# LPengYang/MotionClone

Hardware: NVIDIA H100
Metric: frames/sec at 16x512x512 T2V, 50-step DDIM (higher is better)
Workload: dtype f16

## Files before the change

### motionclone_b200/csrc/spatial_attn_bwd_tc.cu

```cuda
#include <math.h>

#include "tma_common.cuh"

namespace mc {

constexpr int kBM = 128;
constexpr int kBT = 64;

struct FABwdParams {
  const float* lse2;
  const float* dsc;
  __half *dq, *dk, *dv;
  int64_t g_sb, g_sr;
  int B, Nq, Nk, H, Npad;
  float scale, scale_log2e;
};


template <int DH>
__global__ void __launch_bounds__(256) attn_bwd_prep_kernel(const __half* __restrict__ o, const __half* __restrict__ d_o,
                                                            const float* __restrict__ lse, float* __restrict__ lse2,
                                                            float* __restrict__ dsc, int64_t o_sb, int64_t o_sr,
                                                            int64_t do_sb, int64_t do_sr, int B, int N, int Npad, int H,
                                                            float scale) {
  const int64_t i = (int64_t)blockIdx.x * blockDim.x + threadIdx.x;
  if (i >= (int64_t)B * Npad * H) return;
  const int h = (int)(i % H);
  const int64_t br = i / H;
  const int r = (int)(br % Npad), b = (int)(br / Npad);
  const int64_t dst = ((int64_t)b * H + h) * Npad + r;
  if (r >= N) {
    lse2[dst] = 0.f, dsc[dst] = 0.f;
    return;
  }
  const uint4* po = reinterpret_cast<const uint4*>(o + b * o_sb + (int64_t)r * o_sr + h * DH);
  const uint4* pd = reinterpret_cast<const uint4*>(d_o + b * do_sb + (int64_t)r * do_sr + h * DH);
  float acc = 0.f;
#pragma unroll
  for (int c = 0; c < DH / 8; ++c) {
    const uint4 a = po[c], g = pd[c];
    const __half2* ah = reinterpret_cast<const __half2*>(&a);
    const __half2* gh = reinterpret_cast<const __half2*>(&g);
#pragma unroll
    for (int j = 0; j < 4; ++j) {
      const float2 x = __half22float2(ah[j]), y = __half22float2(gh[j]);
      acc = fmaf(x.x, y.x, acc);
      acc = fmaf(x.y, y.y, acc);
    }
  }
  lse2[dst] = lse[((int64_t)b * H + h) * N + r] * 1.44269504088896340736f;
  dsc[dst] = acc * scale;
}


template <int DH>
__device__ __forceinline__ void store_acc_rows(const float* acc, __half* base, int64_t sr, int row0, int nrows, int t) {
#pragma unroll
  for (int r = 0; r < 2; ++r) {
    const int row = row0 + 8 * r;
    if (row >= nrows) continue;
    __half* p = base + (int64_t)row * sr;
#pragma unroll
    for (int i = 0; i < AccW<DH>::REGS / 4; ++i) {
      const int col = 8 * i + 2 * t;
      if (col < DH) *reinterpret_cast<uint32_t*>(p + col) = pack_half2(acc[4 * i + 2 * r], acc[4 * i + 2 * r + 1]);
    }
  }
}

template <int DH, bool SINGLE>
struct DQCfg {
  static constexpr int BN = SINGLE ? kMaxTextKeys : kBT;
  using TQ = TileParts<DH, kBM>;
  using TK = TileParts<DH, BN>;
  static constexpr int ACC = AccW<DH>::REGS;
  static constexpr int NS = SINGLE ? 1 : 2;
  static constexpr int THREADS = 2 * 128 + 32;
  static constexpr int QB = align1k(TQ::BYTES), KB = align1k(TK::BYTES);
  static constexpr int OFF_Q = 0, OFF_DO = QB, OFF_K = 2 * QB, OFF_V = OFF_K + NS * KB, OFF_BAR = OFF_V + NS * KB;
  static constexpr int SMEM = OFF_BAR + 256 + 1024;
};

template <int DH, bool SINGLE, bool RAGGED>
__global__ void __launch_bounds__(DQCfg<DH, SINGLE>::THREADS, 1)
attn_bwd_dq_kernel(const __grid_constant__ CUtensorMap mq128, const __grid_constant__ CUtensorMap mq32,
                   const __grid_constant__ CUtensorMap mdo128, const __grid_constant__ CUtensorMap mdo32,
                   const __grid_constant__ CUtensorMap mk128, const __grid_constant__ CUtensorMap mk32,
                   const __grid_constant__ CUtensorMap mv128, const __grid_constant__ CUtensorMap mv32,
                   const FABwdParams prm) {
  using X = DQCfg<DH, SINGLE>;
  using TQ = typename X::TQ;
  using TK = typename X::TK;
  constexpr int BN = X::BN, NS = X::NS;

  extern __shared__ uint8_t smem_raw[];
  uint8_t* smem = reinterpret_cast<uint8_t*>((reinterpret_cast<uintptr_t>(smem_raw) + 1023) & ~(uintptr_t)1023);
  uint8_t* sQ = smem + X::OFF_Q;
  uint8_t* sDO = smem + X::OFF_DO;
  uint8_t* sK = smem + X::OFF_K;
  uint8_t* sV = smem + X::OFF_V;
  uint64_t* bars = reinterpret_cast<uint64_t*>(smem + X::OFF_BAR);
  uint64_t* bar_q = bars;
  uint64_t* full = bars + 1;
  uint64_t* empty = bars + 1 + NS;

  const int tid = threadIdx.x, warp = tid >> 5, lane = tid & 31;
  const int h = blockIdx.y, b = blockIdx.z;
  const int q0 = blockIdx.x * kBM;
  const int T_tiles = (prm.Nk + BN - 1) / BN;

  if (tid == 0) {
    mbar_init(bar_q, 1);
    for (int i = 0; i < NS; ++i) mbar_init(full + i, 1), mbar_init(empty + i, 8);
    fence_mbar_init();
  }
  __syncthreads();

  if (warp == 8) {
    if (lane == 0) {
      mbar_arrive_expect_tx(bar_q, 2 * TQ::BYTES);
      tma_load_tile<DH, kBM>(sQ, &mq128, &mq32, bar_q, q0, h, b);
      tma_load_tile<DH, kBM>(sDO, &mdo128, &mdo32, bar_q, q0, h, b);
      for (int j = 0; j < T_tiles; ++j) {
        const int st = j % NS;
        if (j >= NS) mbar_wait(empty + st, ((j / NS) - 1) & 1);
        mbar_arrive_expect_tx(full + st, 2 * TK::BYTES);
        tma_load_tile<DH, BN>(sK + st * X::KB, &mk128, &mk32, full + st, j * BN, h, b);
        tma_load_tile<DH, BN>(sV + st * X::KB, &mv128, &mv32, full + st, j * BN, h, b);
      }
    }
    return;
  }

  const int wg = warp >> 2, g = lane >> 2, t = lane & 3;
  const int row0 = q0 + wg * 64 + (warp & 3) * 16 + g;
  const float c = prm.scale_log2e, scale = prm.scale;
  float neg_lse2[2] = {0.f, 0.f}, dscr[2] = {0.f, 0.f};
  if constexpr (!SINGLE) {
    const int64_t base = ((int64_t)b * prm.H + h) * prm.Npad;
#pragma unroll
    for (int r = 0; r < 2; ++r) {
      const int row = row0 + 8 * r;
      if (row < prm.Npad) neg_lse2[r] = -prm.lse2[base + row], dscr[r] = prm.dsc[base + row];
    }
  }
  float dq[X::ACC];
#pragma unroll
  for (int i = 0; i < X::ACC; ++i) dq[i] = 0.f;
  mbar_wait(bar_q, 0);

  for (int j = 0; j < T_tiles; ++j) {
    const int st = j % NS;
    mbar_wait(full + st, (j / NS) & 1);
    float s[BN / 2], dp[BN / 2];
    wg_fence();
    gemm_kk<DH, kBM, BN>(s, smem_u32(sQ), wg * 64, smem_u32(sK + st * X::KB));
    gemm_kk<DH, kBM, BN>(dp, smem_u32(sDO), wg * 64, smem_u32(sV + st * X::KB));
    wg_commit();
    wg_wait<0>();

    if constexpr (SINGLE) {
#pragma unroll
      for (int i = 0; i < BN / 2; ++i)
        if ((i >> 2) * 8 + 2 * t + (i & 1) >= prm.Nk) s[i] = -INFINITY;
#pragma unroll
      for (int r = 0; r < 2; ++r) {
        float mx = -INFINITY;
#pragma unroll
        for (int i = 0; i < BN / 8; ++i) mx = fmaxf(mx, fmaxf(s[4 * i + 2 * r], s[4 * i + 2 * r + 1]));
        mx = fmaxf(mx, __shfl_xor_sync(0xffffffffu, mx, 1));
        mx = fmaxf(mx, __shfl_xor_sync(0xffffffffu, mx, 2));
        const float negm = -mx * c;
        float sum = 0.f;
#pragma unroll
        for (int i = 0; i < BN / 8; ++i)
#pragma unroll
          for (int e = 0; e < 2; ++e) {
            const int k = 4 * i + 2 * r + e;
            s[k] = ex2_approx(fmaf(s[k], c, negm));
            sum += s[k];
          }
        sum += __shfl_xor_sync(0xffffffffu, sum, 1);
        sum += __shfl_xor_sync(0xffffffffu, sum, 2);
        const float inv = 1.f / sum;
        float d = 0.f;
#pragma unroll
        for (int i = 0; i < BN / 8; ++i)
#pragma unroll
          for (int e = 0; e < 2; ++e) {
            const int k = 4 * i + 2 * r + e;
            s[k] *= inv;
            d = fmaf(s[k], dp[k], d);
          }
        d += __shfl_xor_sync(0xffffffffu, d, 1);
        d += __shfl_xor_sync(0xffffffffu, d, 2);
#pragma unroll
        for (int i = 0; i < BN / 8; ++i)
#pragma unroll
          for (int e = 0; e < 2; ++e) {
            const int k = 4 * i + 2 * r + e;
            dp[k] = scale * s[k] * (dp[k] - d);
          }
      }
    } else {
#pragma unroll
      for (int i = 0; i < BN / 2; ++i) {
        const int r = (i >> 1) & 1;
        const float p = ex2_approx(fmaf(s[i], c, neg_lse2[r]));
        dp[i] = p * fmaf(dp[i], scale, -dscr[r]);
      }
      if constexpr (RAGGED) {
        const int kvalid = prm.Nk - j * BN;
        if (kvalid < BN) {
#pragma unroll
          for (int i = 0; i < BN / 2; ++i)
            if ((i >> 2) * 8 + 2 * t + (i & 1) >= kvalid) dp[i] = 0.f;
        }
      }
    }
    uint32_t da[BN / 4];
    acc_to_afrag<BN>(dp, da);
    wg_fence();
    gemm_rmn<DH, BN>(dq, da, smem_u32(sK + st * X::KB));
    wg_commit();
    wg_wait<0>();
    __syncwarp();
    if (lane == 0) mbar_arrive(empty + st);
  }
  store_acc_rows<DH>(dq, prm.dq + (int64_t)b * prm.g_sb + h * DH, prm.g_sr, row0, prm.Nq, t);
}

template <int DH>
struct KVCfg {
  static constexpr int WG = DH > 96 ? 1 : 2;
  static constexpr int KM = WG * 64;
  static constexpr int BT = DH > 96 ? 32 : 64;
  using TK = TileParts<DH, KM>;
  using TQ = TileParts<DH, BT>;
  static constexpr int ACC = AccW<DH>::REGS;
  static constexpr int NS = 2;
  static constexpr int THREADS = WG * 128 + 32;
  static constexpr int KB = align1k(TK::BYTES), QB = align1k(TQ::BYTES);
  static constexpr int OFF_K = 0, OFF_V = KB, OFF_Q = 2 * KB, OFF_DO = OFF_Q + NS * QB, OFF_BAR = OFF_DO + NS * QB;
  static constexpr int SMEM = OFF_BAR + 256 + 1024;
};

template <int DH>
__global__ void __launch_bounds__(KVCfg<DH>::THREADS, 1)
attn_bwd_dkv_kernel(const __grid_constant__ CUtensorMap mk128, const __grid_constant__ CUtensorMap mk32,
                    const __grid_constant__ CUtensorMap mv128, const __grid_constant__ CUtensorMap mv32,
                    const __grid_constant__ CUtensorMap mq128, const __grid_constant__ CUtensorMap mq32,
                    const __grid_constant__ CUtensorMap mdo128, const __grid_constant__ CUtensorMap mdo32,
                    const FABwdParams prm) {
  using X = KVCfg<DH>;
  using TK = typename X::TK;
  using TQ = typename X::TQ;
  constexpr int KM = X::KM, BT = X::BT, NS = X::NS;

  extern __shared__ uint8_t smem_raw[];
  uint8_t* smem = reinterpret_cast<uint8_t*>((reinterpret_cast<uintptr_t>(smem_raw) + 1023) & ~(uintptr_t)1023);
  uint8_t* sK = smem + X::OFF_K;
  uint8_t* sV = smem + X::OFF_V;
  uint8_t* sQ = smem + X::OFF_Q;
  uint8_t* sDO = smem + X::OFF_DO;
  uint64_t* bars = reinterpret_cast<uint64_t*>(smem + X::OFF_BAR);
  uint64_t* bar_kv = bars;
  uint64_t* full = bars + 1;
  uint64_t* empty = bars + 1 + NS;

  const int tid = threadIdx.x, warp = tid >> 5, lane = tid & 31;
  const int h = blockIdx.y, b = blockIdx.z;
  const int k0 = blockIdx.x * KM;
  const int T_tiles = (prm.Nq + BT - 1) / BT;

  if (tid == 0) {
    mbar_init(bar_kv, 1);
    for (int i = 0; i < NS; ++i) mbar_init(full + i, 1), mbar_init(empty + i, X::WG * 4);
    fence_mbar_init();
  }
  __syncthreads();

  if (warp == X::WG * 4) {
    if (lane == 0) {
      mbar_arrive_expect_tx(bar_kv, 2 * TK::BYTES);
      tma_load_tile<DH, KM>(sK, &mk128, &mk32, bar_kv, k0, h, b);
      tma_load_tile<DH, KM>(sV, &mv128, &mv32, bar_kv, k0, h, b);
      for (int j = 0; j < T_tiles; ++j) {
        const int st = j % NS;
        if (j >= NS) mbar_wait(empty + st, ((j / NS) - 1) & 1);
        mbar_arrive_expect_tx(full + st, 2 * TQ::BYTES);
        tma_load_tile<DH, BT>(sQ + st * X::QB, &mq128, &mq32, full + st, j * BT, h, b);
        tma_load_tile<DH, BT>(sDO + st * X::QB, &mdo128, &mdo32, full + st, j * BT, h, b);
      }
    }
    return;
  }

  const int wg = warp >> 2, g = lane >> 2, t = lane & 3;
  const int krow0 = k0 + wg * 64 + (warp & 3) * 16 + g;
  const float c = prm.scale_log2e, scale = prm.scale;
  const float* lse2 = prm.lse2 + ((int64_t)b * prm.H + h) * prm.Npad;
  const float* dsc = prm.dsc + ((int64_t)b * prm.H + h) * prm.Npad;
  float dk[X::ACC], dv[X::ACC];
#pragma unroll
  for (int i = 0; i < X::ACC; ++i) dk[i] = 0.f, dv[i] = 0.f;
  mbar_wait(bar_kv, 0);

  for (int j = 0; j < T_tiles; ++j) {
    const int st = j % NS;
    mbar_wait(full + st, (j / NS) & 1);
    const uint32_t aQ = smem_u32(sQ + st * X::QB), aDO = smem_u32(sDO + st * X::QB);
    float s[BT / 2], dp[BT / 2];
    wg_fence();
    gemm_kk<DH, KM, BT>(s, smem_u32(sK), wg * 64, aQ);
    gemm_kk<DH, KM, BT>(dp, smem_u32(sV), wg * 64, aDO);
    wg_commit();
    wg_wait<0>();
#pragma unroll
    for (int i = 0; i < BT / 8; ++i)
#pragma unroll
      for (int e = 0; e < 2; ++e) {
        const int qc = j * BT + 8 * i + 2 * t + e;
        const float nl = -lse2[qc], d = dsc[qc];
#pragma unroll
        for (int r = 0; r < 2; ++r) {
          const int k = 4 * i + 2 * r + e;
          s[k] = ex2_approx(fmaf(s[k], c, nl));
          dp[k] = s[k] * fmaf(dp[k], scale, -d);
        }
      }
    uint32_t pa[BT / 4], da[BT / 4];
    acc_to_afrag<BT>(s, pa);
    acc_to_afrag<BT>(dp, da);
    wg_fence();
    gemm_rmn<DH, BT>(dv, pa, aDO);
    gemm_rmn<DH, BT>(dk, da, aQ);
    wg_commit();
    wg_wait<0>();
    __syncwarp();
    if (lane == 0) mbar_arrive(empty + st);
  }
  store_acc_rows<DH>(dk, prm.dk + (int64_t)b * prm.g_sb + h * DH, prm.g_sr, krow0, prm.Nk, t);
  store_acc_rows<DH>(dv, prm.dv + (int64_t)b * prm.g_sb + h * DH, prm.g_sr, krow0, prm.Nk, t);
}

template <int DH, bool SINGLE>
static int launch_dq(const AttnMaps& q, const AttnMaps& d_o, const AttnMaps& k, const AttnMaps& v, const FABwdParams& prm,
                     cudaStream_t st) {
  using X = DQCfg<DH, SINGLE>;
  auto kern = attn_bwd_dq_kernel<DH, SINGLE, false>;
  if constexpr (!SINGLE) {
    if (prm.Nk % kBT) kern = attn_bwd_dq_kernel<DH, false, true>;
  }
  cudaFuncSetAttribute(kern, cudaFuncAttributeMaxDynamicSharedMemorySize, X::SMEM);
  dim3 grid((prm.Nq + kBM - 1) / kBM, prm.H, prm.B);
  kern<<<grid, X::THREADS, X::SMEM, st>>>(q.m128, q.m32, d_o.m128, d_o.m32, k.m128, k.m32, v.m128, v.m32, prm);
  count_launch();
  return check_launch(SINGLE ? "cross_attn_bwd_dq" : "spatial_attn_bwd_dq");
}

template <int DH>
static int launch_spatial_bwd(const void* q, const void* k, const void* v, const void* o, const void* d_o, const float* lse,
                              float* workspace, FABwdParams prm, int64_t q_sb, int64_t q_sr, int64_t k_sb, int64_t k_sr,
                              int64_t v_sb, int64_t v_sr, int64_t o_sb, int64_t o_sr, int64_t do_sb, int64_t do_sr,
                              cudaStream_t st) {
  using KV = KVCfg<DH>;
  const int B = prm.B, N = prm.Nq, H = prm.H, Npad = prm.Npad;
  AttnMaps q128, do128, k64, v64, kres, vres, qs, dos;
  int rc = make_attn_maps<DH>(q128, q, H, N, B, q_sr, q_sb, kBM) | make_attn_maps<DH>(do128, d_o, H, N, B, do_sr, do_sb, kBM) |
           make_attn_maps<DH>(k64, k, H, N, B, k_sr, k_sb, kBT) | make_attn_maps<DH>(v64, v, H, N, B, v_sr, v_sb, kBT) |
           make_attn_maps<DH>(kres, k, H, N, B, k_sr, k_sb, KV::KM) | make_attn_maps<DH>(vres, v, H, N, B, v_sr, v_sb, KV::KM) |
           make_attn_maps<DH>(qs, q, H, N, B, q_sr, q_sb, KV::BT) | make_attn_maps<DH>(dos, d_o, H, N, B, do_sr, do_sb, KV::BT);
  if (rc) return MC_E_CUDA;
  float* lse2 = workspace;
  float* dsc = workspace + (int64_t)B * H * Npad;
  prm.lse2 = lse2, prm.dsc = dsc;
  {
    const int64_t total = (int64_t)B * Npad * H;
    attn_bwd_prep_kernel<DH><<<(unsigned)((total + 255) / 256), 256, 0, st>>>((const __half*)o, (const __half*)d_o, lse, lse2,
                                                                            dsc, o_sb, o_sr, do_sb, do_sr, B, N, Npad, H,
                                                                            prm.scale);
    count_launch();
    if (int e = check_launch("attn_bwd_prep")) return e;
  }
  if (int e = launch_dq<DH, false>(q128, do128, k64, v64, prm, st)) return e;
  {
    auto kern = attn_bwd_dkv_kernel<DH>;
    cudaFuncSetAttribute(kern, cudaFuncAttributeMaxDynamicSharedMemorySize, KV::SMEM);
    dim3 grid((N + KV::KM - 1) / KV::KM, H, B);
    kern<<<grid, KV::THREADS, KV::SMEM, st>>>(kres.m128, kres.m32, vres.m128, vres.m32, qs.m128, qs.m32, dos.m128, dos.m32, prm);
    count_launch();
    if (int e = check_launch("spatial_attn_bwd_dkv")) return e;
  }
  return MC_OK;
}

template <int DH>
static int launch_cross_bwd(const void* q, const void* k, const void* v, const void* d_o, const FABwdParams& prm,
                            int64_t q_sb, int64_t q_sr, int64_t kv_sb, int64_t kv_sr, int64_t do_sb, int64_t do_sr,
                            cudaStream_t st) {
  AttnMaps mq, mdo, mk, mv;
  if (make_attn_maps<DH>(mq, q, prm.H, prm.Nq, prm.B, q_sr, q_sb, kBM) ||
      make_attn_maps<DH>(mdo, d_o, prm.H, prm.Nq, prm.B, do_sr, do_sb, kBM) ||
      make_attn_maps<DH>(mk, k, prm.H, prm.Nk, prm.B, kv_sr, kv_sb, kMaxTextKeys) ||
      make_attn_maps<DH>(mv, v, prm.H, prm.Nk, prm.B, kv_sr, kv_sb, kMaxTextKeys))
    return MC_E_CUDA;
  return launch_dq<DH, true>(mq, mdo, mk, mv, prm, st);
}

static inline int npad64(int N) { return (N + 63) / 64 * 64; }

}

extern "C" int64_t mc_spatial_attn_bwd_workspace_bytes(int B, int N, int H) {
  return (int64_t)2 * B * H * mc::npad64(N) * 4;
}

extern "C" int mc_spatial_attn_bwd(const void* q, const void* k, const void* v, const void* o, const void* d_o,
                                   const float* lse, void* dq, void* dk, void* dv, void* workspace, int B, int N, int H,
                                   int DH, int64_t q_stride_b, int64_t q_stride_row, int64_t k_stride_b,
                                   int64_t k_stride_row, int64_t v_stride_b, int64_t v_stride_row, int64_t o_stride_b,
                                   int64_t o_stride_row, int64_t do_stride_b, int64_t do_stride_row, int64_t g_stride_b,
                                   int64_t g_stride_row, float scale, void* stream) {
  using namespace mc;
  if (!q || !k || !v || !o || !d_o || !lse || !dq || !dk || !dv || !workspace || B <= 0 || N <= 0 || H <= 0) {
    set_error("spatial_attn_bwd: null pointer or non-positive dims");
    return MC_E_INVALID;
  }
  if (B > 65535 || H > 65535) {
    set_error("spatial_attn_bwd: at most 65535 frames / heads");
    return MC_E_UNSUPPORTED;
  }
  if ((q_stride_b | q_stride_row | k_stride_b | k_stride_row | v_stride_b | v_stride_row | o_stride_b | o_stride_row |
       do_stride_b | do_stride_row | g_stride_b | g_stride_row) % 8 ||
      ((uintptr_t)q | (uintptr_t)k | (uintptr_t)v | (uintptr_t)o | (uintptr_t)d_o | (uintptr_t)dq | (uintptr_t)dk |
       (uintptr_t)dv | (uintptr_t)workspace) % 16) {
    set_error("spatial_attn_bwd: pointers must be 16-byte aligned and strides multiples of 8 elements");
    return MC_E_INVALID;
  }
  FABwdParams prm{};
  prm.dq = (__half*)dq, prm.dk = (__half*)dk, prm.dv = (__half*)dv, prm.g_sb = g_stride_b, prm.g_sr = g_stride_row;
  prm.B = B, prm.Nq = N, prm.Nk = N, prm.H = H, prm.Npad = npad64(N), prm.scale = scale, prm.scale_log2e = scale * 1.44269504088896340736f;
  cudaStream_t st = (cudaStream_t)stream;
#define MC_SB_CASE(D)                                                                                                      \
  case D:                                                                                                                  \
    return launch_spatial_bwd<D>(q, k, v, o, d_o, lse, (float*)workspace, prm, q_stride_b, q_stride_row, k_stride_b,       \
                                 k_stride_row, v_stride_b, v_stride_row, o_stride_b, o_stride_row, do_stride_b, do_stride_row, st);
  switch (DH) {
    MC_SB_CASE(8) MC_SB_CASE(16) MC_SB_CASE(32) MC_SB_CASE(40) MC_SB_CASE(64) MC_SB_CASE(80) MC_SB_CASE(160)
    default: break;
  }
#undef MC_SB_CASE
  set_error("spatial_attn_bwd: unsupported head dim %d (8, 16, 32, 40, 64, 80, 160)", DH);
  return MC_E_UNSUPPORTED;
}

extern "C" int mc_cross_attn_bwd_dq(const void* q, const void* k, const void* v, const void* d_o, void* dq, int B, int Nq,
                                    int Nk, int H, int DH, int64_t q_stride_b, int64_t q_stride_row, int64_t kv_stride_b,
                                    int64_t kv_stride_row, int64_t do_stride_b, int64_t do_stride_row,
                                    int64_t dq_stride_b, int64_t dq_stride_row, float scale, void* stream) {
  using namespace mc;
  if (!q || !k || !v || !d_o || !dq || B <= 0 || Nq <= 0 || Nk <= 0 || H <= 0) {
    set_error("cross_attn_bwd_dq: null pointer or non-positive dims");
    return MC_E_INVALID;
  }
  if (Nk > kMaxTextKeys) {
    set_error("cross_attn_bwd_dq: at most %d keys (text tokens) per tile, got %d", kMaxTextKeys, Nk);
    return MC_E_UNSUPPORTED;
  }
  if (B > 65535 || H > 65535) {
    set_error("cross_attn_bwd_dq: at most 65535 batches / heads");
    return MC_E_UNSUPPORTED;
  }
  if ((q_stride_row | kv_stride_row | dq_stride_row | q_stride_b | kv_stride_b | dq_stride_b | do_stride_b | do_stride_row) % 8 ||
      ((uintptr_t)q | (uintptr_t)k | (uintptr_t)v | (uintptr_t)d_o | (uintptr_t)dq) % 16) {
    set_error("cross_attn_bwd_dq: pointers must be 16-byte aligned and strides multiples of 8 elements");
    return MC_E_INVALID;
  }
  FABwdParams prm{};
  prm.dq = (__half*)dq, prm.g_sb = dq_stride_b, prm.g_sr = dq_stride_row;
  prm.B = B, prm.Nq = Nq, prm.Nk = Nk, prm.H = H;
  prm.scale = scale, prm.scale_log2e = scale * 1.44269504088896340736f;
  cudaStream_t st = (cudaStream_t)stream;
#define MC_XB_CASE(D)                                                                                                    \
  case D:                                                                                                                \
    return launch_cross_bwd<D>(q, k, v, d_o, prm, q_stride_b, q_stride_row, kv_stride_b, kv_stride_row, do_stride_b,    \
                               do_stride_row, st);
  switch (DH) {
    MC_XB_CASE(8) MC_XB_CASE(16) MC_XB_CASE(32) MC_XB_CASE(40) MC_XB_CASE(64) MC_XB_CASE(80) MC_XB_CASE(160)
    default: break;
  }
#undef MC_XB_CASE
  set_error("cross_attn_bwd_dq: unsupported head dim %d (8, 16, 32, 40, 64, 80, 160)", DH);
  return MC_E_UNSUPPORTED;
}
```

### motionclone_b200/csrc/spatial_attn_tc.cu

```cuda
#include <math.h>

#include "tma_common.cuh"

namespace mc {

constexpr int kFM = 128;
constexpr int kFBN = 64;
constexpr int kFWG = kFM / 64;
constexpr int kFThreads = kFWG * 128 + 32;
constexpr int kFProducerWarp = kFWG * 4;

struct FAParams {
  float* lse;
  __half* o;
  int64_t o_sb, o_sr;
  int B, Nq, Nk, H;
  float scale_log2e;
};

template <int DH>
struct FACfg {
  using TQ = TileParts<DH, kFM>;
  using TK = TileParts<DH, kFBN>;
  static constexpr int ACC = AccW<DH>::REGS;
  static constexpr int NS = DH <= 80 ? 4 : 3;
  static constexpr int QB = align1k(TQ::BYTES), KB = align1k(TK::BYTES);
  static constexpr int OFF_Q = 0, OFF_K = QB, OFF_V = OFF_K + NS * KB, OFF_BAR = OFF_V + NS * KB;
  static constexpr int SMEM = OFF_BAR + 256 + 1024;
};

template <int DH>
__global__ void __launch_bounds__(kFThreads, 1)
attn_fwd_kernel(const __grid_constant__ CUtensorMap mq128, const __grid_constant__ CUtensorMap mk128,
                const __grid_constant__ CUtensorMap mv128, const __grid_constant__ CUtensorMap mq32,
                const __grid_constant__ CUtensorMap mk32, const __grid_constant__ CUtensorMap mv32, const FAParams prm) {
  using X = FACfg<DH>;
  using TQ = typename X::TQ;
  using TK = typename X::TK;
  constexpr int BN = kFBN, NS = X::NS;

  extern __shared__ uint8_t smem_raw[];
  uint8_t* smem = reinterpret_cast<uint8_t*>((reinterpret_cast<uintptr_t>(smem_raw) + 1023) & ~(uintptr_t)1023);
  uint8_t* sQ = smem + X::OFF_Q;
  uint8_t* sK = smem + X::OFF_K;
  uint8_t* sV = smem + X::OFF_V;
  uint64_t* bars = reinterpret_cast<uint64_t*>(smem + X::OFF_BAR);
  uint64_t* bar_q = bars;
  uint64_t* full = bars + 1;
  uint64_t* empty = bars + 1 + NS;

  const int tid = threadIdx.x, warp = tid >> 5, lane = tid & 31;
  const int h = blockIdx.y, b = blockIdx.z;
  const int q0 = blockIdx.x * kFM;
  const int T_tiles = (prm.Nk + BN - 1) / BN;

  if (tid == 0) {
    mbar_init(bar_q, 1);
    for (int i = 0; i < NS; ++i) mbar_init(full + i, 1), mbar_init(empty + i, kFWG * 4);
    fence_mbar_init();
  }
  __syncthreads();

  if (warp == kFProducerWarp) {
    if (lane == 0) {
      tma_prefetch_desc(&mq128), tma_prefetch_desc(&mk128), tma_prefetch_desc(&mv128);
      mbar_arrive_expect_tx(bar_q, TQ::BYTES);
      tma_load_tile<DH, kFM>(sQ, &mq128, &mq32, bar_q, q0, h, b);
      for (int j = 0; j < T_tiles; ++j) {
        const int st = j % NS;
        if (j >= NS) mbar_wait(empty + st, ((j / NS) - 1) & 1);
        mbar_arrive_expect_tx(full + st, 2 * TK::BYTES);
        tma_load_tile<DH, BN>(sK + st * X::KB, &mk128, &mk32, full + st, j * BN, h, b);
        tma_load_tile<DH, BN>(sV + st * X::KB, &mv128, &mv32, full + st, j * BN, h, b);
      }
    }
    return;
  }

  const int wg = warp >> 2, g = lane >> 2, t = lane & 3;
  const int row0 = q0 + wg * 64 + (warp & 3) * 16 + g;
  const float c = prm.scale_log2e;
  float o[X::ACC];
#pragma unroll
  for (int i = 0; i < X::ACC; ++i) o[i] = 0.f;
  float m_[2] = {-INFINITY, -INFINITY}, l_[2] = {0.f, 0.f};
  mbar_wait(bar_q, 0);
  const uint32_t aQ = smem_u32(sQ);

  for (int j = 0; j < T_tiles; ++j) {
    const int st = j % NS;
    mbar_wait(full + st, (j / NS) & 1);
    float s[BN / 2];
    wg_fence();
    gemm_kk<DH, kFM, BN>(s, aQ, wg * 64, smem_u32(sK + st * X::KB));
    wg_commit();
    wg_wait<0>();

    const int kvalid = prm.Nk - j * BN;
    if (kvalid < BN) {
#pragma unroll
      for (int i = 0; i < BN / 2; ++i)
        if ((i >> 2) * 8 + 2 * t + (i & 1) >= kvalid) s[i] = -INFINITY;
    }
    float negm[2];
#pragma unroll
    for (int r = 0; r < 2; ++r) {
      float mx = -INFINITY;
#pragma unroll
      for (int i = 0; i < BN / 8; ++i) mx = fmaxf(mx, fmaxf(s[4 * i + 2 * r], s[4 * i + 2 * r + 1]));
      mx = fmaxf(mx, __shfl_xor_sync(0xffffffffu, mx, 1));
      mx = fmaxf(mx, __shfl_xor_sync(0xffffffffu, mx, 2));
      const float m_new = fmaxf(m_[r], mx * c);
      const float alpha = ex2_approx(m_[r] - m_new);
      m_[r] = m_new;
      l_[r] *= alpha;
#pragma unroll
      for (int i = 0; i < X::ACC / 4; ++i) o[4 * i + 2 * r] *= alpha, o[4 * i + 2 * r + 1] *= alpha;
      negm[r] = -m_new;
    }
#pragma unroll
    for (int i = 0; i < BN / 8; ++i) {
#pragma unroll
      for (int r = 0; r < 2; ++r) {
        float p0, p1;
        ex2_pair(i, s[4 * i + 2 * r], s[4 * i + 2 * r + 1], c, negm[r], p0, p1);
        l_[r] += p0 + p1;
        s[4 * i + 2 * r] = p0, s[4 * i + 2 * r + 1] = p1;
      }
    }
    uint32_t pa[BN / 4];
    acc_to_afrag<BN>(s, pa);
    wg_fence();
    gemm_rmn<DH, BN>(o, pa, smem_u32(sV + st * X::KB));
    wg_commit();
    wg_wait<0>();
    __syncwarp();
    if (lane == 0) mbar_arrive(empty + st);
  }

#pragma unroll
  for (int r = 0; r < 2; ++r) {
    float l = l_[r];
    l += __shfl_xor_sync(0xffffffffu, l, 1);
    l += __shfl_xor_sync(0xffffffffu, l, 2);
    const float inv = 1.f / l;
    const int row = row0 + 8 * r;
    if (row < prm.Nq) {
      __half* orow = prm.o + (int64_t)b * prm.o_sb + (int64_t)row * prm.o_sr + h * DH;
#pragma unroll
      for (int i = 0; i < X::ACC / 4; ++i) {
        const int col = 8 * i + 2 * t;
        if (col < DH) *reinterpret_cast<uint32_t*>(orow + col) = pack_half2(o[4 * i + 2 * r] * inv, o[4 * i + 2 * r + 1] * inv);
      }
      if (prm.lse != nullptr && t == 0) prm.lse[((int64_t)b * prm.H + h) * prm.Nq + row] = (m_[r] + log2f(l)) * 0.6931471805599453f;
    }
  }
}

template <int DH>
static int launch_attn_fwd(const void* q, const void* k, const void* v, const FAParams& prm, int64_t q_sb, int64_t q_sr,
                           int64_t k_sb, int64_t k_sr, int64_t v_sb, int64_t v_sr, cudaStream_t st) {
  using X = FACfg<DH>;
  AttnMaps mq, mk, mv;
  if (make_attn_maps<DH>(mq, q, prm.H, prm.Nq, prm.B, q_sr, q_sb, kFM) ||
      make_attn_maps<DH>(mk, k, prm.H, prm.Nk, prm.B, k_sr, k_sb, kFBN) ||
      make_attn_maps<DH>(mv, v, prm.H, prm.Nk, prm.B, v_sr, v_sb, kFBN)) {
    return MC_E_CUDA;
  }
  const int q_tiles = (prm.Nq + kFM - 1) / kFM;
  auto kern = attn_fwd_kernel<DH>;
  cudaFuncSetAttribute(kern, cudaFuncAttributeMaxDynamicSharedMemorySize, X::SMEM);
  dim3 grid(q_tiles, prm.H, prm.B);
  kern<<<grid, kFThreads, X::SMEM, st>>>(mq.m128, mk.m128, mv.m128, mq.m32, mk.m32, mv.m32, prm);
  count_launch();
  return check_launch("attn_fwd");
}

static int attn_fwd_dispatch(const char* what, int DH, const void* q, const void* k, const void* v, const FAParams& prm,
                             int64_t q_sb, int64_t q_sr, int64_t k_sb, int64_t k_sr, int64_t v_sb, int64_t v_sr,
                             cudaStream_t st) {
#define MC_FA_CASE(D) \
  case D: return launch_attn_fwd<D>(q, k, v, prm, q_sb, q_sr, k_sb, k_sr, v_sb, v_sr, st);
  switch (DH) {
    MC_FA_CASE(8) MC_FA_CASE(16) MC_FA_CASE(32) MC_FA_CASE(40) MC_FA_CASE(64) MC_FA_CASE(80) MC_FA_CASE(160)
    default: break;
  }
#undef MC_FA_CASE
  set_error("%s: unsupported head dim %d (8, 16, 32, 40, 64, 80, 160)", what, DH);
  return MC_E_UNSUPPORTED;
}

}

extern "C" int mc_spatial_attn_fwd(const void* q, const void* k, const void* v, void* o, float* lse, int B, int N, int H,
                                   int DH, int64_t q_stride_b, int64_t q_stride_row, int64_t k_stride_b,
                                   int64_t k_stride_row, int64_t v_stride_b, int64_t v_stride_row, int64_t o_stride_b,
                                   int64_t o_stride_row, float scale, void* stream) {
  using namespace mc;
  if (!q || !k || !v || !o || B <= 0 || N <= 0 || H <= 0) {
    set_error("spatial_attn_fwd: null pointer or non-positive dims");
    return MC_E_INVALID;
  }
  if (B > 65535 || H > 65535) {
    set_error("spatial_attn_fwd: at most 65535 frames / heads");
    return MC_E_UNSUPPORTED;
  }
  if ((q_stride_b | q_stride_row | k_stride_b | k_stride_row | v_stride_b | v_stride_row | o_stride_b | o_stride_row) % 8 ||
      ((uintptr_t)q | (uintptr_t)k | (uintptr_t)v | (uintptr_t)o) % 16) {
    set_error("spatial_attn_fwd: pointers must be 16-byte aligned and strides multiples of 8 elements");
    return MC_E_INVALID;
  }
  FAParams prm{};
  prm.lse = lse, prm.o = (__half*)o, prm.o_sb = o_stride_b, prm.o_sr = o_stride_row;
  prm.B = B, prm.Nq = N, prm.Nk = N, prm.H = H;
  prm.scale_log2e = scale * 1.44269504088896340736f;
  return attn_fwd_dispatch("spatial_attn_fwd", DH, q, k, v, prm, q_stride_b, q_stride_row, k_stride_b, k_stride_row,
                           v_stride_b, v_stride_row, (cudaStream_t)stream);
}

extern "C" int mc_cross_attn_fwd(const void* q, const void* k, const void* v, void* o, int B, int Nq, int Nk, int H, int DH,
                                 int64_t q_stride_b, int64_t q_stride_row, int64_t kv_stride_b, int64_t kv_stride_row,
                                 int64_t o_stride_b, int64_t o_stride_row, float scale, void* stream) {
  using namespace mc;
  if (!q || !k || !v || !o || B <= 0 || Nq <= 0 || Nk <= 0 || H <= 0) {
    set_error("cross_attn_fwd: null pointer or non-positive dims");
    return MC_E_INVALID;
  }
  if (Nk > kMaxTextKeys) {
    set_error("cross_attn_fwd: at most %d keys (text tokens), got %d", kMaxTextKeys, Nk);
    return MC_E_UNSUPPORTED;
  }
  if (B > 65535 || H > 65535) {
    set_error("cross_attn_fwd: at most 65535 batches / heads");
    return MC_E_UNSUPPORTED;
  }
  if ((q_stride_row | kv_stride_row | o_stride_row | q_stride_b | kv_stride_b | o_stride_b) % 8 ||
      ((uintptr_t)q | (uintptr_t)k | (uintptr_t)v | (uintptr_t)o) % 16) {
    set_error("cross_attn_fwd: pointers must be 16-byte aligned and strides multiples of 8 elements");
    return MC_E_INVALID;
  }
  FAParams prm{};
  prm.lse = nullptr, prm.o = (__half*)o, prm.o_sb = o_stride_b, prm.o_sr = o_stride_row;
  prm.B = B, prm.Nq = Nq, prm.Nk = Nk, prm.H = H;
  prm.scale_log2e = scale * 1.44269504088896340736f;
  return attn_fwd_dispatch("cross_attn_fwd", DH, q, k, v, prm, q_stride_b, q_stride_row, kv_stride_b, kv_stride_row,
                           kv_stride_b, kv_stride_row, (cudaStream_t)stream);
}
```

### motionclone_b200/csrc/tc_common.cuh

```cuda
#pragma once
#include "mc_common.cuh"

namespace mc {

__device__ __forceinline__ void wgmma_ss_n32(float* d, uint64_t a, uint64_t b, int accum) {
  asm volatile(
      "{\n.reg .pred p;\nsetp.ne.b32 p, %18, 0;\n"
      "wgmma.mma_async.sync.aligned.m64n32k16.f32.f16.f16 {%0,%1,%2,%3,%4,%5,%6,%7,%8,%9,%10,%11,%12,%13,%14,%15}, %16, %17, p, 1, 1, 0, 0;\n}\n"
      : "+f"(d[0]), "+f"(d[1]), "+f"(d[2]), "+f"(d[3]), "+f"(d[4]), "+f"(d[5]), "+f"(d[6]), "+f"(d[7]), "+f"(d[8]), "+f"(d[9]), "+f"(d[10]), "+f"(d[11]), "+f"(d[12]), "+f"(d[13]), "+f"(d[14]), "+f"(d[15])
      : "l"(a), "l"(b), "r"(accum));
}
__device__ __forceinline__ void wgmma_ss_n64(float* d, uint64_t a, uint64_t b, int accum) {
  asm volatile(
      "{\n.reg .pred p;\nsetp.ne.b32 p, %34, 0;\n"
      "wgmma.mma_async.sync.aligned.m64n64k16.f32.f16.f16 {%0,%1,%2,%3,%4,%5,%6,%7,%8,%9,%10,%11,%12,%13,%14,%15,%16,%17,%18,%19,%20,%21,%22,%23,%24,%25,%26,%27,%28,%29,%30,%31}, %32, %33, p, 1, 1, 0, 0;\n}\n"
      : "+f"(d[0]), "+f"(d[1]), "+f"(d[2]), "+f"(d[3]), "+f"(d[4]), "+f"(d[5]), "+f"(d[6]), "+f"(d[7]), "+f"(d[8]), "+f"(d[9]), "+f"(d[10]), "+f"(d[11]), "+f"(d[12]), "+f"(d[13]), "+f"(d[14]), "+f"(d[15]), "+f"(d[16]), "+f"(d[17]), "+f"(d[18]), "+f"(d[19]), "+f"(d[20]), "+f"(d[21]), "+f"(d[22]), "+f"(d[23]), "+f"(d[24]), "+f"(d[25]), "+f"(d[26]), "+f"(d[27]), "+f"(d[28]), "+f"(d[29]), "+f"(d[30]), "+f"(d[31])
      : "l"(a), "l"(b), "r"(accum));
}
__device__ __forceinline__ void wgmma_ss_n80(float* d, uint64_t a, uint64_t b, int accum) {
  asm volatile(
      "{\n.reg .pred p;\nsetp.ne.b32 p, %42, 0;\n"
      "wgmma.mma_async.sync.aligned.m64n80k16.f32.f16.f16 {%0,%1,%2,%3,%4,%5,%6,%7,%8,%9,%10,%11,%12,%13,%14,%15,%16,%17,%18,%19,%20,%21,%22,%23,%24,%25,%26,%27,%28,%29,%30,%31,%32,%33,%34,%35,%36,%37,%38,%39}, %40, %41, p, 1, 1, 0, 0;\n}\n"
      : "+f"(d[0]), "+f"(d[1]), "+f"(d[2]), "+f"(d[3]), "+f"(d[4]), "+f"(d[5]), "+f"(d[6]), "+f"(d[7]), "+f"(d[8]), "+f"(d[9]), "+f"(d[10]), "+f"(d[11]), "+f"(d[12]), "+f"(d[13]), "+f"(d[14]), "+f"(d[15]), "+f"(d[16]), "+f"(d[17]), "+f"(d[18]), "+f"(d[19]), "+f"(d[20]), "+f"(d[21]), "+f"(d[22]), "+f"(d[23]), "+f"(d[24]), "+f"(d[25]), "+f"(d[26]), "+f"(d[27]), "+f"(d[28]), "+f"(d[29]), "+f"(d[30]), "+f"(d[31]), "+f"(d[32]), "+f"(d[33]), "+f"(d[34]), "+f"(d[35]), "+f"(d[36]), "+f"(d[37]), "+f"(d[38]), "+f"(d[39])
      : "l"(a), "l"(b), "r"(accum));
}
__device__ __forceinline__ void wgmma_rs_n16(float* d, const uint32_t* a, uint64_t b, int accum) {
  asm volatile(
      "{\n.reg .pred p;\nsetp.ne.b32 p, %13, 0;\n"
      "wgmma.mma_async.sync.aligned.m64n16k16.f32.f16.f16 {%0,%1,%2,%3,%4,%5,%6,%7}, {%8,%9,%10,%11}, %12, p, 1, 1, 1;\n}\n"
      : "+f"(d[0]), "+f"(d[1]), "+f"(d[2]), "+f"(d[3]), "+f"(d[4]), "+f"(d[5]), "+f"(d[6]), "+f"(d[7])
      : "r"(a[0]), "r"(a[1]), "r"(a[2]), "r"(a[3]), "l"(b), "r"(accum));
}
__device__ __forceinline__ void wgmma_rs_n64(float* d, const uint32_t* a, uint64_t b, int accum) {
  asm volatile(
      "{\n.reg .pred p;\nsetp.ne.b32 p, %37, 0;\n"
      "wgmma.mma_async.sync.aligned.m64n64k16.f32.f16.f16 {%0,%1,%2,%3,%4,%5,%6,%7,%8,%9,%10,%11,%12,%13,%14,%15,%16,%17,%18,%19,%20,%21,%22,%23,%24,%25,%26,%27,%28,%29,%30,%31}, {%32,%33,%34,%35}, %36, p, 1, 1, 1;\n}\n"
      : "+f"(d[0]), "+f"(d[1]), "+f"(d[2]), "+f"(d[3]), "+f"(d[4]), "+f"(d[5]), "+f"(d[6]), "+f"(d[7]), "+f"(d[8]), "+f"(d[9]), "+f"(d[10]), "+f"(d[11]), "+f"(d[12]), "+f"(d[13]), "+f"(d[14]), "+f"(d[15]), "+f"(d[16]), "+f"(d[17]), "+f"(d[18]), "+f"(d[19]), "+f"(d[20]), "+f"(d[21]), "+f"(d[22]), "+f"(d[23]), "+f"(d[24]), "+f"(d[25]), "+f"(d[26]), "+f"(d[27]), "+f"(d[28]), "+f"(d[29]), "+f"(d[30]), "+f"(d[31])
      : "r"(a[0]), "r"(a[1]), "r"(a[2]), "r"(a[3]), "l"(b), "r"(accum));
}

template <int N>
__device__ __forceinline__ void wgmma_ss(float* d, uint64_t a, uint64_t b, int accum) {
  static_assert(N == 32 || N == 64 || N == 80, "wgmma_ss: N in {32, 64, 80}");
  if constexpr (N == 32) wgmma_ss_n32(d, a, b, accum);
  else if constexpr (N == 64) wgmma_ss_n64(d, a, b, accum);
  else wgmma_ss_n80(d, a, b, accum);
}
template <int N>
__device__ __forceinline__ void wgmma_rs(float* d, const uint32_t* a, uint64_t b, int accum) {
  static_assert(N == 16 || N == 64, "wgmma_rs: N in {16, 64}");
  if constexpr (N == 16) wgmma_rs_n16(d, a, b, accum);
  else wgmma_rs_n64(d, a, b, accum);
}

__device__ __forceinline__ void wg_fence() { asm volatile("wgmma.fence.sync.aligned;" ::: "memory"); }
__device__ __forceinline__ void wg_commit() { asm volatile("wgmma.commit_group.sync.aligned;" ::: "memory"); }
template <int PENDING>
__device__ __forceinline__ void wg_wait() { asm volatile("wgmma.wait_group.sync.aligned %0;" ::"n"(PENDING) : "memory"); }

__device__ __forceinline__ uint64_t gmma_desc(uint32_t saddr, uint32_t lbo_bytes, uint32_t sbo_bytes, uint32_t layout) {
  uint64_t d = 0;
  d |= (uint64_t)((saddr & 0x3FFFFu) >> 4);
  d |= (uint64_t)((lbo_bytes >> 4) & 0x3FFFu) << 16;
  d |= (uint64_t)((sbo_bytes >> 4) & 0x3FFFu) << 32;
  d |= (uint64_t)layout << 62;
  return d;
}

template <int KR>
__device__ __forceinline__ void acc_to_afrag(const float* s, uint32_t* a) {
#pragma unroll
  for (int i = 0; i < KR / 2; i += 2) a[i / 2] = pack_half2(s[i], s[i + 1]);
}

}
```

### motionclone_b200/csrc/tma_common.cuh

```cuda
#pragma once
#include <cuda.h>

#include "tc_common.cuh"

namespace mc {

typedef CUresult (*mc_encode_tiled_fn)(CUtensorMap*, CUtensorMapDataType, cuuint32_t, void*, const cuuint64_t*,
                                       const cuuint64_t*, const cuuint32_t*, const cuuint32_t*, CUtensorMapInterleave,
                                       CUtensorMapSwizzle, CUtensorMapL2promotion, CUtensorMapFloatOOBfill);

inline mc_encode_tiled_fn tensor_map_encoder() {
  static mc_encode_tiled_fn fn = [] {
    void* p = nullptr;
    cudaDriverEntryPointQueryResult q;
    if (cudaGetDriverEntryPoint("cuTensorMapEncodeTiled", &p, cudaEnableDefault, &q) != cudaSuccess ||
        q != cudaDriverEntryPointSuccess)
      p = nullptr;
    return (mc_encode_tiled_fn)p;
  }();
  return fn;
}

inline int make_attn_tensor_map(CUtensorMap* map, const void* base, int DH, int H, int64_t rows, int64_t frames,
                                int64_t stride_r, int64_t stride_b, int box_e, int box_rows, bool swizzle128) {
  mc_encode_tiled_fn enc = tensor_map_encoder();
  static thread_local bool ctx_bound = false;
  if (!ctx_bound) {
    cudaFree(nullptr);
    ctx_bound = true;
  }
  if (!enc) {
    set_error("cuTensorMapEncodeTiled: driver entry point unavailable (cudaGetDriverEntryPoint failed)");
    return -1;
  }
  cuuint64_t gdim[4] = {(cuuint64_t)DH, (cuuint64_t)H, (cuuint64_t)rows, (cuuint64_t)frames};
  cuuint64_t gstr[3] = {(cuuint64_t)DH * 2, (cuuint64_t)stride_r * 2, (cuuint64_t)stride_b * 2};
  if (frames == 1) gstr[2] = gstr[1] * (cuuint64_t)rows;
  cuuint32_t box[4] = {(cuuint32_t)box_e, 1u, (cuuint32_t)box_rows, 1u};
  cuuint32_t estr[4] = {1u, 1u, 1u, 1u};
  CUresult r = enc(map, CU_TENSOR_MAP_DATA_TYPE_FLOAT16, 4, const_cast<void*>(base), gdim, gstr, box, estr,
                   CU_TENSOR_MAP_INTERLEAVE_NONE, swizzle128 ? CU_TENSOR_MAP_SWIZZLE_128B : CU_TENSOR_MAP_SWIZZLE_32B,
                   CU_TENSOR_MAP_L2_PROMOTION_L2_128B, CU_TENSOR_MAP_FLOAT_OOB_FILL_NONE);
  if (r != CUDA_SUCCESS)
    set_error("cuTensorMapEncodeTiled -> CUresult %d: base %p dims (%d, %d, %lld, %lld) strides (%lld, %lld) elements, box "
              "(%d, 1, %d, 1), swizzle %s", (int)r, base, DH, H, (long long)rows, (long long)frames, (long long)stride_r,
              (long long)stride_b, box_e, box_rows, swizzle128 ? "128B" : "32B");
  return r == CUDA_SUCCESS ? 0 : (int)r;
}

constexpr int kMaxTextKeys = 80;

struct AttnMaps {
  CUtensorMap m128, m32;
};
template <int DH>
int make_attn_maps(AttnMaps& m, const void* base, int H, int N, int B, int64_t sr, int64_t sb, int rows) {
  int rc = make_attn_tensor_map(&m.m128, base, DH, H, N, B, sr, sb, 64, rows, true);
  if (rc) return rc;
  if (DH >= 64 && DH % 64 != 0) rc = make_attn_tensor_map(&m.m32, base, DH, H, N, B, sr, sb, 16, rows, false);
  else m.m32 = m.m128;
  return rc;
}

__device__ __forceinline__ void tma_load_4d(void* sdst, const CUtensorMap* map, uint64_t* bar, int c0, int c1, int c2,
                                            int c3) {
  asm volatile(
      "cp.async.bulk.tensor.4d.shared::cluster.global.tile.mbarrier::complete_tx::bytes [%0], [%1, {%3, %4, %5, %6}], [%2];"
      ::"r"(smem_u32(sdst)), "l"(map), "r"(smem_u32(bar)), "r"(c0), "r"(c1), "r"(c2), "r"(c3)
      : "memory");
}
__device__ __forceinline__ void tma_prefetch_desc(const CUtensorMap* map) {
  asm volatile("prefetch.tensormap [%0];" ::"l"(map) : "memory");
}

template <int DH, int ROWS = 128>
struct TileParts {
  static_assert(DH % 8 == 0, "head dim must be a multiple of 8 (16-byte rows)");
  static_assert(ROWS % 8 == 0 && ROWS <= 256, "tile rows");
  static constexpr int N64 = DH >= 64 ? DH / 64 : 1;
  static constexpr int REM = DH >= 64 ? DH % 64 : 0;
  static_assert(REM % 16 == 0, "head dims above 64 must be 64*a + 16*b");
  static constexpr int N16 = REM / 16;
  static constexpr int DHP = DH >= 64 ? DH : (DH + 15) / 16 * 16;
  static constexpr int KS64 = DH >= 64 ? 4 : DHP / 16;
  static constexpr int W64 = DH >= 64 ? 64 : DHP;
  static constexpr int P64 = ROWS * 128, P16 = ROWS * 32;
  static constexpr int BYTES = N64 * P64 + N16 * P16;
  static constexpr int KSTEPS = N64 * KS64 + N16;
  __host__ __device__ static constexpr int part64_off(int p) { return p * P64; }
  __host__ __device__ static constexpr int part16_off(int p) { return N64 * P64 + p * P16; }
};

template <int DH, int ROWS = 128>
__device__ __forceinline__ void tma_load_tile(uint8_t* sdst, const CUtensorMap* map128, const CUtensorMap* map32,
                                              uint64_t* bar, int r0, int h, int b) {
  using T = TileParts<DH, ROWS>;
#pragma unroll
  for (int p = 0; p < T::N64; ++p) tma_load_4d(sdst + T::part64_off(p), map128, bar, p * 64, h, r0, b);
#pragma unroll
  for (int p = 0; p < T::N16; ++p) tma_load_4d(sdst + T::part16_off(p), map32, bar, T::N64 * 64 + p * 16, h, r0, b);
}

__device__ __forceinline__ uint64_t desc_k128(uint32_t part_addr, int ks) { return gmma_desc(part_addr + ks * 32, 16, 1024, 1); }
__device__ __forceinline__ uint64_t desc_k32(uint32_t part_addr) { return gmma_desc(part_addr, 16, 256, 3); }
__device__ __forceinline__ uint64_t desc_mn128(uint32_t part_addr, int ks) { return gmma_desc(part_addr + ks * 2048, 16384, 1024, 1); }
__device__ __forceinline__ uint64_t desc_mn32(uint32_t part_addr, int ks) { return gmma_desc(part_addr + ks * 512, 4096, 256, 3); }

__host__ __device__ constexpr int align1k(int bytes) { return (bytes + 1023) / 1024 * 1024; }

template <int DH, int AROWS, int BN>
__device__ __forceinline__ void gemm_kk(float* d, uint32_t sA, int arow0, uint32_t sB) {
  using TA = TileParts<DH, AROWS>;
  using TB = TileParts<DH, BN>;
  int acc = 0;
#pragma unroll
  for (int p = 0; p < TA::N64; ++p)
#pragma unroll
    for (int ks = 0; ks < TA::KS64; ++ks) {
      wgmma_ss<BN>(d, desc_k128(sA + TA::part64_off(p) + arow0 * 128, ks), desc_k128(sB + TB::part64_off(p), ks), acc);
      acc = 1;
    }
#pragma unroll
  for (int p = 0; p < TA::N16; ++p) {
    wgmma_ss<BN>(d, desc_k32(sA + TA::part16_off(p) + arow0 * 32), desc_k32(sB + TB::part16_off(p)), acc);
    acc = 1;
  }
}

template <int DH>
struct AccW {
  using T = TileParts<DH, 64>;
  static constexpr int W = T::N64 * 64 + T::N16 * 16;
  static constexpr int REGS = W / 2;
};
template <int DH, int KR>
__device__ __forceinline__ void gemm_rmn(float* d, const uint32_t* a, uint32_t sB) {
  using TB = TileParts<DH, KR>;
#pragma unroll
  for (int ks = 0; ks < KR / 16; ++ks) {
#pragma unroll
    for (int p = 0; p < TB::N64; ++p) wgmma_rs<64>(d + p * 32, a + 4 * ks, desc_mn128(sB + TB::part64_off(p), ks), 1);
#pragma unroll
    for (int p = 0; p < TB::N16; ++p)
      wgmma_rs<16>(d + TB::N64 * 32 + p * 8, a + 4 * ks, desc_mn32(sB + TB::part16_off(p), ks), 1);
  }
}

__device__ __forceinline__ float ex2_approx(float x) {
  float y;
  asm("ex2.approx.ftz.f32 %0, %1;" : "=f"(y) : "f"(x));
  return y;
}

__device__ __forceinline__ float ex2_poly(float s, float c, float negm) {
  constexpr float k4 = 0.009570101276040077f;
  constexpr float k3 = 0.05591786280274391f;
  constexpr float k2 = 0.240247443318367f;
  constexpr float k1 = 0.6931217908859253f;
  constexpr float k0 = 0.9999992847442627f;
  const float x = fmaxf(fmaf(s, c, negm), -126.f);
  const float t = __fadd_rn(x, 12582912.f);
  const float f = __fsub_rn(x, __fadd_rn(t, -12582912.f));
  float p = fmaf(k4, f, k3);
  p = fmaf(p, f, k2);
  p = fmaf(p, f, k1);
  p = fmaf(p, f, k0);
  return __uint_as_float(__float_as_uint(p) + (__float_as_uint(t) << 23));
}
#ifndef MC_EX2_POLY_PERIOD
#define MC_EX2_POLY_PERIOD 4
#endif
__device__ __forceinline__ void ex2_pair(int pair_index, float s0, float s1, float c, float negm, float& p0, float& p1) {
  if (MC_EX2_POLY_PERIOD > 0 && pair_index % (MC_EX2_POLY_PERIOD > 0 ? MC_EX2_POLY_PERIOD : 1) == (MC_EX2_POLY_PERIOD - 1)) {
    p0 = ex2_poly(s0, c, negm);
    p1 = ex2_poly(s1, c, negm);
  } else {
    p0 = ex2_approx(fmaf(s0, c, negm));
    p1 = ex2_approx(fmaf(s1, c, negm));
  }
}

}
```

Baseline: 2.521.

## Add narrow head-dim tiling and pipelined forward attention for DH 40/80

Adds a NARROW tile layout for head dims below 64. It stores only 16-column parts instead of padding to a 64-wide part, and uses a single m64n48 wgmma for the PV/dQ products. The backward dq/dkv kernels get narrow variants used when DH==40, and a new forward kernel with a 4-stage TMA pipeline (4 warpgroups for narrow dims) serves DH 40 and 80. The aim is to cut wasted padding bytes and MMA work for small head dims and to overlap loads better. In exchange it adds new descriptor strides and layouts that must match TMA boxes exactly.

```diff
diff --git a/motionclone_b200/csrc/spatial_attn_bwd_tc.cu b/motionclone_b200/csrc/spatial_attn_bwd_tc.cu
--- a/motionclone_b200/csrc/spatial_attn_bwd_tc.cu
+++ b/motionclone_b200/csrc/spatial_attn_bwd_tc.cu
@@ -53,7 +53,7 @@
 }
 
 
-template <int DH>
+template <int DH, bool NW = false>
 __device__ __forceinline__ void store_acc_rows(const float* acc, __half* base, int64_t sr, int row0, int nrows, int t) {
 #pragma unroll
   for (int r = 0; r < 2; ++r) {
@@ -61,19 +61,19 @@
     if (row >= nrows) continue;
     __half* p = base + (int64_t)row * sr;
 #pragma unroll
-    for (int i = 0; i < AccW<DH>::REGS / 4; ++i) {
+    for (int i = 0; i < AccW<DH, NW>::REGS / 4; ++i) {
       const int col = 8 * i + 2 * t;
       if (col < DH) *reinterpret_cast<uint32_t*>(p + col) = pack_half2(acc[4 * i + 2 * r], acc[4 * i + 2 * r + 1]);
     }
   }
 }
 
-template <int DH, bool SINGLE>
+template <int DH, bool SINGLE, bool NW = false>
 struct DQCfg {
   static constexpr int BN = SINGLE ? kMaxTextKeys : kBT;
-  using TQ = TileParts<DH, kBM>;
-  using TK = TileParts<DH, BN>;
-  static constexpr int ACC = AccW<DH>::REGS;
+  using TQ = TileParts<DH, kBM, NW>;
+  using TK = TileParts<DH, BN, NW>;
+  static constexpr int ACC = AccW<DH, NW>::REGS;
   static constexpr int NS = SINGLE ? 1 : 2;
   static constexpr int THREADS = 2 * 128 + 32;
   static constexpr int QB = align1k(TQ::BYTES), KB = align1k(TK::BYTES);
@@ -81,14 +81,13 @@
   static constexpr int SMEM = OFF_BAR + 256 + 1024;
 };
 
-template <int DH, bool SINGLE, bool RAGGED>
-__global__ void __launch_bounds__(DQCfg<DH, SINGLE>::THREADS, 1)
-attn_bwd_dq_kernel(const __grid_constant__ CUtensorMap mq128, const __grid_constant__ CUtensorMap mq32,
-                   const __grid_constant__ CUtensorMap mdo128, const __grid_constant__ CUtensorMap mdo32,
-                   const __grid_constant__ CUtensorMap mk128, const __grid_constant__ CUtensorMap mk32,
-                   const __grid_constant__ CUtensorMap mv128, const __grid_constant__ CUtensorMap mv32,
-                   const FABwdParams prm) {
-  using X = DQCfg<DH, SINGLE>;
+template <int DH, bool SINGLE, bool RAGGED, bool NW>
+__device__ __forceinline__ void attn_bwd_dq_body(const CUtensorMap& mq128, const CUtensorMap& mq32,
+                                                 const CUtensorMap& mdo128, const CUtensorMap& mdo32,
+                                                 const CUtensorMap& mk128, const CUtensorMap& mk32,
+                                                 const CUtensorMap& mv128, const CUtensorMap& mv32,
+                                                 const FABwdParams& prm) {
+  using X = DQCfg<DH, SINGLE, NW>;
   using TQ = typename X::TQ;
   using TK = typename X::TK;
   constexpr int BN = X::BN, NS = X::NS;
@@ -119,14 +118,14 @@
   if (warp == 8) {
     if (lane == 0) {
       mbar_arrive_expect_tx(bar_q, 2 * TQ::BYTES);
-      tma_load_tile<DH, kBM>(sQ, &mq128, &mq32, bar_q, q0, h, b);
-      tma_load_tile<DH, kBM>(sDO, &mdo128, &mdo32, bar_q, q0, h, b);
+      tma_load_tile<DH, kBM, NW>(sQ, &mq128, &mq32, bar_q, q0, h, b);
+      tma_load_tile<DH, kBM, NW>(sDO, &mdo128, &mdo32, bar_q, q0, h, b);
       for (int j = 0; j < T_tiles; ++j) {
         const int st = j % NS;
         if (j >= NS) mbar_wait(empty + st, ((j / NS) - 1) & 1);
         mbar_arrive_expect_tx(full + st, 2 * TK::BYTES);
-        tma_load_tile<DH, BN>(sK + st * X::KB, &mk128, &mk32, full + st, j * BN, h, b);
-        tma_load_tile<DH, BN>(sV + st * X::KB, &mv128, &mv32, full + st, j * BN, h, b);
+        tma_load_tile<DH, BN, NW>(sK + st * X::KB, &mk128, &mk32, full + st, j * BN, h, b);
+        tma_load_tile<DH, BN, NW>(sV + st * X::KB, &mv128, &mv32, full + st, j * BN, h, b);
       }
     }
     return;
@@ -154,8 +153,8 @@
     mbar_wait(full + st, (j / NS) & 1);
     float s[BN / 2], dp[BN / 2];
     wg_fence();
-    gemm_kk<DH, kBM, BN>(s, smem_u32(sQ), wg * 64, smem_u32(sK + st * X::KB));
-    gemm_kk<DH, kBM, BN>(dp, smem_u32(sDO), wg * 64, smem_u32(sV + st * X::KB));
+    gemm_kk<DH, kBM, BN, NW>(s, smem_u32(sQ), wg * 64, smem_u32(sK + st * X::KB));
+    gemm_kk<DH, kBM, BN, NW>(dp, smem_u32(sDO), wg * 64, smem_u32(sV + st * X::KB));
     wg_commit();
     wg_wait<0>();
 
@@ -221,23 +220,43 @@
     uint32_t da[BN / 4];
     acc_to_afrag<BN>(dp, da);
     wg_fence();
-    gemm_rmn<DH, BN>(dq, da, smem_u32(sK + st * X::KB));
+    gemm_rmn<DH, BN, NW>(dq, da, smem_u32(sK + st * X::KB));
     wg_commit();
     wg_wait<0>();
     __syncwarp();
     if (lane == 0) mbar_arrive(empty + st);
   }
-  store_acc_rows<DH>(dq, prm.dq + (int64_t)b * prm.g_sb + h * DH, prm.g_sr, row0, prm.Nq, t);
-}
-
-template <int DH>
+  store_acc_rows<DH, NW>(dq, prm.dq + (int64_t)b * prm.g_sb + h * DH, prm.g_sr, row0, prm.Nq, t);
+}
+
+template <int DH, bool SINGLE, bool RAGGED>
+__global__ void __launch_bounds__(DQCfg<DH, SINGLE>::THREADS, 1)
+attn_bwd_dq_kernel(const __grid_constant__ CUtensorMap mq128, const __grid_constant__ CUtensorMap mq32,
+                   const __grid_constant__ CUtensorMap mdo128, const __grid_constant__ CUtensorMap mdo32,
+                   const __grid_constant__ CUtensorMap mk128, const __grid_constant__ CUtensorMap mk32,
+                   const __grid_constant__ CUtensorMap mv128, const __grid_constant__ CUtensorMap mv32,
+                   const FABwdParams prm) {
+  attn_bwd_dq_body<DH, SINGLE, RAGGED, false>(mq128, mq32, mdo128, mdo32, mk128, mk32, mv128, mv32, prm);
+}
+
+template <int DH, bool RAGGED>
+__global__ void __launch_bounds__(DQCfg<DH, false>::THREADS, 1)
+attn_bwd_dq_narrow_kernel(const __grid_constant__ CUtensorMap mq128, const __grid_constant__ CUtensorMap mq32,
+                          const __grid_constant__ CUtensorMap mdo128, const __grid_constant__ CUtensorMap mdo32,
+                          const __grid_constant__ CUtensorMap mk128, const __grid_constant__ CUtensorMap mk32,
+                          const __grid_constant__ CUtensorMap mv128, const __grid_constant__ CUtensorMap mv32,
+                          const FABwdParams prm) {
+  attn_bwd_dq_body<DH, false, RAGGED, true>(mq128, mq32, mdo128, mdo32, mk128, mk32, mv128, mv32, prm);
+}
+
+template <int DH, bool NW = false>
 struct KVCfg {
   static constexpr int WG = DH > 96 ? 1 : 2;
   static constexpr int KM = WG * 64;
   static constexpr int BT = DH > 96 ? 32 : 64;
-  using TK = TileParts<DH, KM>;
-  using TQ = TileParts<DH, BT>;
-  static constexpr int ACC = AccW<DH>::REGS;
+  using TK = TileParts<DH, KM, NW>;
+  using TQ = TileParts<DH, BT, NW>;
+  static constexpr int ACC = AccW<DH, NW>::REGS;
   static constexpr int NS = 2;
   static constexpr int THREADS = WG * 128 + 32;
   static constexpr int KB = align1k(TK::BYTES), QB = align1k(TQ::BYTES);
@@ -245,14 +264,13 @@
   static constexpr int SMEM = OFF_BAR + 256 + 1024;
 };
 
-template <int DH>
-__global__ void __launch_bounds__(KVCfg<DH>::THREADS, 1)
-attn_bwd_dkv_kernel(const __grid_constant__ CUtensorMap mk128, const __grid_constant__ CUtensorMap mk32,
-                    const __grid_constant__ CUtensorMap mv128, const __grid_constant__ CUtensorMap mv32,
-                    const __grid_constant__ CUtensorMap mq128, const __grid_constant__ CUtensorMap mq32,
-                    const __grid_constant__ CUtensorMap mdo128, const __grid_constant__ CUtensorMap mdo32,
-                    const FABwdParams prm) {
-  using X = KVCfg<DH>;
+template <int DH, bool NW>
+__device__ __forceinline__ void attn_bwd_dkv_body(const CUtensorMap& mk128, const CUtensorMap& mk32,
+                                                  const CUtensorMap& mv128, const CUtensorMap& mv32,
+                                                  const CUtensorMap& mq128, const CUtensorMap& mq32,
+                                                  const CUtensorMap& mdo128, const CUtensorMap& mdo32,
+                                                  const FABwdParams& prm) {
+  using X = KVCfg<DH, NW>;
   using TK = typename X::TK;
   using TQ = typename X::TQ;
   constexpr int KM = X::KM, BT = X::BT, NS = X::NS;
@@ -283,14 +301,14 @@
   if (warp == X::WG * 4) {
     if (lane == 0) {
       mbar_arrive_expect_tx(bar_kv, 2 * TK::BYTES);
-      tma_load_tile<DH, KM>(sK, &mk128, &mk32, bar_kv, k0, h, b);
-      tma_load_tile<DH, KM>(sV, &mv128, &mv32, bar_kv, k0, h, b);
+      tma_load_tile<DH, KM, NW>(sK, &mk128, &mk32, bar_kv, k0, h, b);
+      tma_load_tile<DH, KM, NW>(sV, &mv128, &mv32, bar_kv, k0, h, b);
       for (int j = 0; j < T_tiles; ++j) {
         const int st = j % NS;
         if (j >= NS) mbar_wait(empty + st, ((j / NS) - 1) & 1);
         mbar_arrive_expect_tx(full + st, 2 * TQ::BYTES);
-        tma_load_tile<DH, BT>(sQ + st * X::QB, &mq128, &mq32, full + st, j * BT, h, b);
-        tma_load_tile<DH, BT>(sDO + st * X::QB, &mdo128, &mdo32, full + st, j * BT, h, b);
+        tma_load_tile<DH, BT, NW>(sQ + st * X::QB, &mq128, &mq32, full + st, j * BT, h, b);
+        tma_load_tile<DH, BT, NW>(sDO + st * X::QB, &mdo128, &mdo32, full + st, j * BT, h, b);
       }
     }
     return;
@@ -312,8 +330,8 @@
     const uint32_t aQ = smem_u32(sQ + st * X::QB), aDO = smem_u32(sDO + st * X::QB);
     float s[BT / 2], dp[BT / 2];
     wg_fence();
-    gemm_kk<DH, KM, BT>(s, smem_u32(sK), wg * 64, aQ);
-    gemm_kk<DH, KM, BT>(dp, smem_u32(sV), wg * 64, aDO);
+    gemm_kk<DH, KM, BT, NW>(s, smem_u32(sK), wg * 64, aQ);
+    gemm_kk<DH, KM, BT, NW>(dp, smem_u32(sV), wg * 64, aDO);
     wg_commit();
     wg_wait<0>();
 #pragma unroll
@@ -333,25 +351,47 @@
     acc_to_afrag<BT>(s, pa);
     acc_to_afrag<BT>(dp, da);
     wg_fence();
-    gemm_rmn<DH, BT>(dv, pa, aDO);
-    gemm_rmn<DH, BT>(dk, da, aQ);
+    gemm_rmn<DH, BT, NW>(dv, pa, aDO);
+    gemm_rmn<DH, BT, NW>(dk, da, aQ);
     wg_commit();
     wg_wait<0>();
     __syncwarp();
     if (lane == 0) mbar_arrive(empty + st);
   }
-  store_acc_rows<DH>(dk, prm.dk + (int64_t)b * prm.g_sb + h * DH, prm.g_sr, krow0, prm.Nk, t);
-  store_acc_rows<DH>(dv, prm.dv + (int64_t)b * prm.g_sb + h * DH, prm.g_sr, krow0, prm.Nk, t);
-}
-
-template <int DH, bool SINGLE>
+  store_acc_rows<DH, NW>(dk, prm.dk + (int64_t)b * prm.g_sb + h * DH, prm.g_sr, krow0, prm.Nk, t);
+  store_acc_rows<DH, NW>(dv, prm.dv + (int64_t)b * prm.g_sb + h * DH, prm.g_sr, krow0, prm.Nk, t);
+}
+
+template <int DH>
+__global__ void __launch_bounds__(KVCfg<DH>::THREADS, 1)
+attn_bwd_dkv_kernel(const __grid_constant__ CUtensorMap mk128, const __grid_constant__ CUtensorMap mk32,
+                    const __grid_constant__ CUtensorMap mv128, const __grid_constant__ CUtensorMap mv32,
+                    const __grid_constant__ CUtensorMap mq128, const __grid_constant__ CUtensorMap mq32,
+                    const __grid_constant__ CUtensorMap mdo128, const __grid_constant__ CUtensorMap mdo32,
+                    const FABwdParams prm) {
+  attn_bwd_dkv_body<DH, false>(mk128, mk32, mv128, mv32, mq128, mq32, mdo128, mdo32, prm);
+}
+
+template <int DH>
+__global__ void __launch_bounds__(KVCfg<DH, true>::THREADS, 1)
+attn_bwd_dkv_narrow_kernel(const __grid_constant__ CUtensorMap mk128, const __grid_constant__ CUtensorMap mk32,
+                           const __grid_constant__ CUtensorMap mv128, const __grid_constant__ CUtensorMap mv32,
+                           const __grid_constant__ CUtensorMap mq128, const __grid_constant__ CUtensorMap mq32,
+                           const __grid_constant__ CUtensorMap mdo128, const __grid_constant__ CUtensorMap mdo32,
+                           const FABwdParams prm) {
+  attn_bwd_dkv_body<DH, true>(mk128, mk32, mv128, mv32, mq128, mq32, mdo128, mdo32, prm);
+}
+
+template <int DH, bool SINGLE, bool NW = false>
 static int launch_dq(const AttnMaps& q, const AttnMaps& d_o, const AttnMaps& k, const AttnMaps& v, const FABwdParams& prm,
                      cudaStream_t st) {
-  using X = DQCfg<DH, SINGLE>;
-  auto kern = attn_bwd_dq_kernel<DH, SINGLE, false>;
-  if constexpr (!SINGLE) {
-    if (prm.Nk % kBT) kern = attn_bwd_dq_kernel<DH, false, true>;
-  }
+  using X = DQCfg<DH, SINGLE, NW>;
+  const bool ragged = prm.Nk % kBT != 0;
+  auto kern = [ragged] {
+    if constexpr (NW) return ragged ? attn_bwd_dq_narrow_kernel<DH, true> : attn_bwd_dq_narrow_kernel<DH, false>;
+    else if constexpr (SINGLE) return attn_bwd_dq_kernel<DH, true, false>;
+    else return ragged ? attn_bwd_dq_kernel<DH, false, true> : attn_bwd_dq_kernel<DH, false, false>;
+  }();
   cudaFuncSetAttribute(kern, cudaFuncAttributeMaxDynamicSharedMemorySize, X::SMEM);
   dim3 grid((prm.Nq + kBM - 1) / kBM, prm.H, prm.B);
   kern<<<grid, X::THREADS, X::SMEM, st>>>(q.m128, q.m32, d_o.m128, d_o.m32, k.m128, k.m32, v.m128, v.m32, prm);
@@ -364,13 +404,17 @@
                               float* workspace, FABwdParams prm, int64_t q_sb, int64_t q_sr, int64_t k_sb, int64_t k_sr,
                               int64_t v_sb, int64_t v_sr, int64_t o_sb, int64_t o_sr, int64_t do_sb, int64_t do_sr,
                               cudaStream_t st) {
-  using KV = KVCfg<DH>;
+  constexpr bool NW = DH == 40;
+  using KV = KVCfg<DH, NW>;
   const int B = prm.B, N = prm.Nq, H = prm.H, Npad = prm.Npad;
   AttnMaps q128, do128, k64, v64, kres, vres, qs, dos;
-  int rc = make_attn_maps<DH>(q128, q, H, N, B, q_sr, q_sb, kBM) | make_attn_maps<DH>(do128, d_o, H, N, B, do_sr, do_sb, kBM) |
-           make_attn_maps<DH>(k64, k, H, N, B, k_sr, k_sb, kBT) | make_attn_maps<DH>(v64, v, H, N, B, v_sr, v_sb, kBT) |
-           make_attn_maps<DH>(kres, k, H, N, B, k_sr, k_sb, KV::KM) | make_attn_maps<DH>(vres, v, H, N, B, v_sr, v_sb, KV::KM) |
-           make_attn_maps<DH>(qs, q, H, N, B, q_sr, q_sb, KV::BT) | make_attn_maps<DH>(dos, d_o, H, N, B, do_sr, do_sb, KV::BT);
+  int rc = make_attn_maps<DH, NW>(q128, q, H, N, B, q_sr, q_sb, kBM) |
+           make_attn_maps<DH, NW>(do128, d_o, H, N, B, do_sr, do_sb, kBM) |
+           make_attn_maps<DH, NW>(k64, k, H, N, B, k_sr, k_sb, kBT) | make_attn_maps<DH, NW>(v64, v, H, N, B, v_sr, v_sb, kBT) |
+           make_attn_maps<DH, NW>(kres, k, H, N, B, k_sr, k_sb, KV::KM) |
+           make_attn_maps<DH, NW>(vres, v, H, N, B, v_sr, v_sb, KV::KM) |
+           make_attn_maps<DH, NW>(qs, q, H, N, B, q_sr, q_sb, KV::BT) |
+           make_attn_maps<DH, NW>(dos, d_o, H, N, B, do_sr, do_sb, KV::BT);
   if (rc) return MC_E_CUDA;
   float* lse2 = workspace;
   float* dsc = workspace + (int64_t)B * H * Npad;
@@ -383,9 +427,12 @@
     count_launch();
     if (int e = check_launch("attn_bwd_prep")) return e;
   }
-  if (int e = launch_dq<DH, false>(q128, do128, k64, v64, prm, st)) return e;
+  if (int e = launch_dq<DH, false, NW>(q128, do128, k64, v64, prm, st)) return e;
   {
-    auto kern = attn_bwd_dkv_kernel<DH>;
+    auto kern = [] {
+      if constexpr (NW) return attn_bwd_dkv_narrow_kernel<DH>;
+      else return attn_bwd_dkv_kernel<DH>;
+    }();
     cudaFuncSetAttribute(kern, cudaFuncAttributeMaxDynamicSharedMemorySize, KV::SMEM);
     dim3 grid((N + KV::KM - 1) / KV::KM, H, B);
     kern<<<grid, KV::THREADS, KV::SMEM, st>>>(kres.m128, kres.m32, vres.m128, vres.m32, qs.m128, qs.m32, dos.m128, dos.m32, prm);
diff --git a/motionclone_b200/csrc/spatial_attn_tc.cu b/motionclone_b200/csrc/spatial_attn_tc.cu
--- a/motionclone_b200/csrc/spatial_attn_tc.cu
+++ b/motionclone_b200/csrc/spatial_attn_tc.cu
@@ -158,6 +158,179 @@
 }
 
 template <int DH>
+struct FAPCfg {
+  static constexpr bool NW = DH < 64;
+  static constexpr int WG = NW ? 4 : 2, M = WG * 64;
+  static constexpr bool SPLIT = WG > 2;
+  static constexpr int THREADS = WG * 128 + (SPLIT ? 128 : 32);
+  using TQ = TileParts<DH, M, NW>;
+  using TK = TileParts<DH, kFBN, NW>;
+  static constexpr int ACC = AccW<DH, NW>::REGS;
+  static constexpr int NS = 4;
+  static constexpr int QB = align1k(TQ::BYTES), KB = align1k(TK::BYTES);
+  static constexpr int OFF_K = QB, OFF_V = OFF_K + NS * KB, OFF_BAR = OFF_V + NS * KB;
+  static constexpr int SMEM = OFF_BAR + 256 + 1024;
+};
+
+template <int DH>
+__global__ void __launch_bounds__(FAPCfg<DH>::THREADS, 1)
+attn_fwd_pipelined_kernel(const __grid_constant__ CUtensorMap mq128, const __grid_constant__ CUtensorMap mk128,
+                          const __grid_constant__ CUtensorMap mv128, const __grid_constant__ CUtensorMap mq32,
+                          const __grid_constant__ CUtensorMap mk32, const __grid_constant__ CUtensorMap mv32,
+                          const FAParams prm) {
+  using X = FAPCfg<DH>;
+  using TQ = typename X::TQ;
+  using TK = typename X::TK;
+  constexpr bool NW = X::NW;
+  constexpr int BN = kFBN, NS = X::NS, ACC = X::ACC, KB = X::KB;
+
+  extern __shared__ uint8_t smem_raw[];
+  uint8_t* smem = reinterpret_cast<uint8_t*>((reinterpret_cast<uintptr_t>(smem_raw) + 1023) & ~(uintptr_t)1023);
+  uint8_t* sQ = smem;
+  uint8_t* sK = smem + X::OFF_K;
+  uint8_t* sV = smem + X::OFF_V;
+  uint64_t* bars = reinterpret_cast<uint64_t*>(smem + X::OFF_BAR);
+  uint64_t* bar_q = bars;
+  uint64_t* full = bars + 1;
+  uint64_t* empty = bars + 1 + NS;
+
+  const int tid = threadIdx.x, warp = tid >> 5, lane = tid & 31;
+  const int h = blockIdx.y, b = blockIdx.z;
+  const int q0 = blockIdx.x * X::M;
+  const int T_tiles = (prm.Nk + BN - 1) / BN;
+
+  if (tid == 0) {
+    mbar_init(bar_q, 1);
+    for (int i = 0; i < NS; ++i) mbar_init(full + i, 1), mbar_init(empty + i, X::WG * 4);
+    fence_mbar_init();
+  }
+  __syncthreads();
+
+  if (warp >= X::WG * 4) {
+    if constexpr (X::SPLIT) asm volatile("setmaxnreg.dec.sync.aligned.u32 40;\n" ::: "memory");
+    if (warp == X::WG * 4 && lane == 0) {
+      tma_prefetch_desc(&mq32), tma_prefetch_desc(&mk32), tma_prefetch_desc(&mv32);
+      mbar_arrive_expect_tx(bar_q, TQ::BYTES);
+      tma_load_tile<DH, X::M, NW>(sQ, &mq128, &mq32, bar_q, q0, h, b);
+      for (int j = 0; j < T_tiles; ++j) {
+        const int st = j % NS;
+        if (j >= NS) mbar_wait(empty + st, ((j / NS) - 1) & 1);
+        mbar_arrive_expect_tx(full + st, 2 * TK::BYTES);
+        tma_load_tile<DH, BN, NW>(sK + st * KB, &mk128, &mk32, full + st, j * BN, h, b);
+        tma_load_tile<DH, BN, NW>(sV + st * KB, &mv128, &mv32, full + st, j * BN, h, b);
+      }
+    }
+    return;
+  }
+
+  if constexpr (X::SPLIT) asm volatile("setmaxnreg.inc.sync.aligned.u32 104;\n" ::: "memory");
+  const int wg = warp >> 2, g = lane >> 2, t = lane & 3;
+  const int row0 = q0 + wg * 64 + (warp & 3) * 16 + g;
+  const float c = prm.scale_log2e;
+  float o[ACC];
+#pragma unroll
+  for (int i = 0; i < ACC; ++i) o[i] = 0.f;
+  float m_[2] = {-INFINITY, -INFINITY}, l_[2] = {0.f, 0.f};
+  mbar_wait(bar_q, 0);
+  const uint32_t aQ = smem_u32(sQ);
+
+  auto softmax = [&](const float* acc, int jj, float* s, float* alpha) {
+#pragma unroll
+    for (int i = 0; i < BN / 2; ++i) s[i] = acc[i];
+    const int kvalid = prm.Nk - jj * BN;
+    if (kvalid < BN) {
+#pragma unroll
+      for (int i = 0; i < BN / 2; ++i)
+        if ((i >> 2) * 8 + 2 * t + (i & 1) >= kvalid) s[i] = -INFINITY;
+    }
+    float negm[2];
+#pragma unroll
+    for (int r = 0; r < 2; ++r) {
+      float mx = -INFINITY;
+#pragma unroll
+      for (int i = 0; i < BN / 8; ++i) mx = fmaxf(mx, fmaxf(s[4 * i + 2 * r], s[4 * i + 2 * r + 1]));
+      mx = fmaxf(mx, __shfl_xor_sync(0xffffffffu, mx, 1));
+      mx = fmaxf(mx, __shfl_xor_sync(0xffffffffu, mx, 2));
+      const float m_new = fmaxf(m_[r], mx * c);
+      alpha[r] = ex2_approx(m_[r] - m_new);
+      m_[r] = m_new;
+      l_[r] *= alpha[r];
+      negm[r] = -m_new;
+    }
+#pragma unroll
+    for (int i = 0; i < BN / 8; ++i) {
+#pragma unroll
+      for (int r = 0; r < 2; ++r) {
+        float p0, p1;
+        ex2_pair(i, s[4 * i + 2 * r], s[4 * i + 2 * r + 1], c, negm[r], p0, p1);
+        l_[r] += p0 + p1;
+        s[4 * i + 2 * r] = p0, s[4 * i + 2 * r + 1] = p1;
+      }
+    }
+  };
+
+  uint32_t pa[BN / 4];
+  {
+    float s[BN / 2], p[BN / 2], alpha[2];
+    mbar_wait(full, 0);
+    wg_fence();
+    gemm_kk<DH, X::M, BN, NW>(s, aQ, wg * 64, smem_u32(sK));
+    wg_commit();
+    wg_wait<0>();
+    softmax(s, 0, p, alpha);
+    acc_to_afrag<BN>(p, pa);
+  }
+  for (int j = 0; j + 1 < T_tiles; ++j) {
+    const int st = j % NS, sn = (j + 1) % NS;
+    mbar_wait(full + sn, ((j + 1) / NS) & 1);
+    float s[BN / 2];
+    wg_fence();
+    gemm_kk<DH, X::M, BN, NW>(s, aQ, wg * 64, smem_u32(sK + sn * KB));
+    wg_commit();
+    gemm_rmn<DH, BN, NW>(o, pa, smem_u32(sV + st * KB));
+    wg_commit();
+    wg_wait<1>();
+    float p[BN / 2], alpha[2];
+    softmax(s, j + 1, p, alpha);
+    wg_wait<0>();
+    __syncwarp();
+    if (lane == 0) mbar_arrive(empty + st);
+#pragma unroll
+    for (int r = 0; r < 2; ++r)
+#pragma unroll
+      for (int i = 0; i < ACC / 4; ++i) o[4 * i + 2 * r] *= alpha[r], o[4 * i + 2 * r + 1] *= alpha[r];
+    acc_to_afrag<BN>(p, pa);
+  }
+  {
+    const int st = (T_tiles - 1) % NS;
+    wg_fence();
+    gemm_rmn<DH, BN, NW>(o, pa, smem_u32(sV + st * KB));
+    wg_commit();
+    wg_wait<0>();
+    __syncwarp();
+    if (lane == 0) mbar_arrive(empty + st);
+  }
+
+#pragma unroll
+  for (int r = 0; r < 2; ++r) {
+    float l = l_[r];
+    l += __shfl_xor_sync(0xffffffffu, l, 1);
+    l += __shfl_xor_sync(0xffffffffu, l, 2);
+    const float inv = 1.f / l;
+    const int row = row0 + 8 * r;
+    if (row < prm.Nq) {
+      __half* orow = prm.o + (int64_t)b * prm.o_sb + (int64_t)row * prm.o_sr + h * DH;
+#pragma unroll
+      for (int i = 0; i < ACC / 4; ++i) {
+        const int col = 8 * i + 2 * t;
+        if (col < DH) *reinterpret_cast<uint32_t*>(orow + col) = pack_half2(o[4 * i + 2 * r] * inv, o[4 * i + 2 * r + 1] * inv);
+      }
+      if (prm.lse != nullptr && t == 0) prm.lse[((int64_t)b * prm.H + h) * prm.Nq + row] = (m_[r] + log2f(l)) * 0.6931471805599453f;
+    }
+  }
+}
+
+template <int DH>
 static int launch_attn_fwd(const void* q, const void* k, const void* v, const FAParams& prm, int64_t q_sb, int64_t q_sr,
                            int64_t k_sb, int64_t k_sr, int64_t v_sb, int64_t v_sr, cudaStream_t st) {
   using X = FACfg<DH>;
@@ -176,6 +349,25 @@
   return check_launch("attn_fwd");
 }
 
+template <int DH>
+static int launch_attn_fwd_pipelined(const void* q, const void* k, const void* v, const FAParams& prm, int64_t q_sb,
+                                     int64_t q_sr, int64_t k_sb, int64_t k_sr, int64_t v_sb, int64_t v_sr, cudaStream_t st) {
+  using X = FAPCfg<DH>;
+  constexpr bool NW = X::NW;
+  AttnMaps mq, mk, mv;
+  if (make_attn_maps<DH, NW>(mq, q, prm.H, prm.Nq, prm.B, q_sr, q_sb, X::M) ||
+      make_attn_maps<DH, NW>(mk, k, prm.H, prm.Nk, prm.B, k_sr, k_sb, kFBN) ||
+      make_attn_maps<DH, NW>(mv, v, prm.H, prm.Nk, prm.B, v_sr, v_sb, kFBN)) {
+    return MC_E_CUDA;
+  }
+  auto kern = attn_fwd_pipelined_kernel<DH>;
+  cudaFuncSetAttribute(kern, cudaFuncAttributeMaxDynamicSharedMemorySize, X::SMEM);
+  dim3 grid((prm.Nq + X::M - 1) / X::M, prm.H, prm.B);
+  kern<<<grid, FAPCfg<DH>::THREADS, X::SMEM, st>>>(mq.m128, mk.m128, mv.m128, mq.m32, mk.m32, mv.m32, prm);
+  count_launch();
+  return check_launch("spatial_attn_fwd");
+}
+
 static int attn_fwd_dispatch(const char* what, int DH, const void* q, const void* k, const void* v, const FAParams& prm,
                              int64_t q_sb, int64_t q_sr, int64_t k_sb, int64_t k_sr, int64_t v_sb, int64_t v_sr,
                              cudaStream_t st) {
@@ -214,6 +406,12 @@
   prm.lse = lse, prm.o = (__half*)o, prm.o_sb = o_stride_b, prm.o_sr = o_stride_row;
   prm.B = B, prm.Nq = N, prm.Nk = N, prm.H = H;
   prm.scale_log2e = scale * 1.44269504088896340736f;
+  if (DH == 40)
+    return launch_attn_fwd_pipelined<40>(q, k, v, prm, q_stride_b, q_stride_row, k_stride_b, k_stride_row, v_stride_b,
+                                         v_stride_row, (cudaStream_t)stream);
+  if (DH == 80)
+    return launch_attn_fwd_pipelined<80>(q, k, v, prm, q_stride_b, q_stride_row, k_stride_b, k_stride_row, v_stride_b,
+                                         v_stride_row, (cudaStream_t)stream);
   return attn_fwd_dispatch("spatial_attn_fwd", DH, q, k, v, prm, q_stride_b, q_stride_row, k_stride_b, k_stride_row,
                            v_stride_b, v_stride_row, (cudaStream_t)stream);
 }
diff --git a/motionclone_b200/csrc/tc_common.cuh b/motionclone_b200/csrc/tc_common.cuh
--- a/motionclone_b200/csrc/tc_common.cuh
+++ b/motionclone_b200/csrc/tc_common.cuh
@@ -31,6 +31,13 @@
       : "+f"(d[0]), "+f"(d[1]), "+f"(d[2]), "+f"(d[3]), "+f"(d[4]), "+f"(d[5]), "+f"(d[6]), "+f"(d[7])
       : "r"(a[0]), "r"(a[1]), "r"(a[2]), "r"(a[3]), "l"(b), "r"(accum));
 }
+__device__ __forceinline__ void wgmma_rs_n48(float* d, const uint32_t* a, uint64_t b, int accum) {
+  asm volatile(
+      "{\n.reg .pred p;\nsetp.ne.b32 p, %29, 0;\n"
+      "wgmma.mma_async.sync.aligned.m64n48k16.f32.f16.f16 {%0,%1,%2,%3,%4,%5,%6,%7,%8,%9,%10,%11,%12,%13,%14,%15,%16,%17,%18,%19,%20,%21,%22,%23}, {%24,%25,%26,%27}, %28, p, 1, 1, 1;\n}\n"
+      : "+f"(d[0]), "+f"(d[1]), "+f"(d[2]), "+f"(d[3]), "+f"(d[4]), "+f"(d[5]), "+f"(d[6]), "+f"(d[7]), "+f"(d[8]), "+f"(d[9]), "+f"(d[10]), "+f"(d[11]), "+f"(d[12]), "+f"(d[13]), "+f"(d[14]), "+f"(d[15]), "+f"(d[16]), "+f"(d[17]), "+f"(d[18]), "+f"(d[19]), "+f"(d[20]), "+f"(d[21]), "+f"(d[22]), "+f"(d[23])
+      : "r"(a[0]), "r"(a[1]), "r"(a[2]), "r"(a[3]), "l"(b), "r"(accum));
+}
 __device__ __forceinline__ void wgmma_rs_n64(float* d, const uint32_t* a, uint64_t b, int accum) {
   asm volatile(
       "{\n.reg .pred p;\nsetp.ne.b32 p, %37, 0;\n"
@@ -48,8 +55,9 @@
 }
 template <int N>
 __device__ __forceinline__ void wgmma_rs(float* d, const uint32_t* a, uint64_t b, int accum) {
-  static_assert(N == 16 || N == 64, "wgmma_rs: N in {16, 64}");
+  static_assert(N == 16 || N == 48 || N == 64, "wgmma_rs: N in {16, 48, 64}");
   if constexpr (N == 16) wgmma_rs_n16(d, a, b, accum);
+  else if constexpr (N == 48) wgmma_rs_n48(d, a, b, accum);
   else wgmma_rs_n64(d, a, b, accum);
 }
 
diff --git a/motionclone_b200/csrc/tma_common.cuh b/motionclone_b200/csrc/tma_common.cuh
--- a/motionclone_b200/csrc/tma_common.cuh
+++ b/motionclone_b200/csrc/tma_common.cuh
@@ -53,8 +53,14 @@
 struct AttnMaps {
   CUtensorMap m128, m32;
 };
-template <int DH>
+template <int DH, bool NARROW = false>
 int make_attn_maps(AttnMaps& m, const void* base, int H, int N, int B, int64_t sr, int64_t sb, int rows) {
+  if constexpr (NARROW) {
+    static_assert(DH < 64, "NARROW: head dims below 64");
+    const int rc = make_attn_tensor_map(&m.m32, base, DH, H, N, B, sr, sb, 16, rows, false);
+    m.m128 = m.m32;
+    return rc;
+  }
   int rc = make_attn_tensor_map(&m.m128, base, DH, H, N, B, sr, sb, 64, rows, true);
   if (rc) return rc;
   if (DH >= 64 && DH % 64 != 0) rc = make_attn_tensor_map(&m.m32, base, DH, H, N, B, sr, sb, 16, rows, false);
@@ -73,12 +79,13 @@
   asm volatile("prefetch.tensormap [%0];" ::"l"(map) : "memory");
 }
 
-template <int DH, int ROWS = 128>
+template <int DH, int ROWS = 128, bool NARROW = false>
 struct TileParts {
   static_assert(DH % 8 == 0, "head dim must be a multiple of 8 (16-byte rows)");
   static_assert(ROWS % 8 == 0 && ROWS <= 256, "tile rows");
-  static constexpr int N64 = DH >= 64 ? DH / 64 : 1;
-  static constexpr int REM = DH >= 64 ? DH % 64 : 0;
+  static_assert(!NARROW || DH < 64, "NARROW: head dims below 64");
+  static constexpr int N64 = NARROW ? 0 : DH >= 64 ? DH / 64 : 1;
+  static constexpr int REM = NARROW ? (DH + 15) / 16 * 16 : DH >= 64 ? DH % 64 : 0;
   static_assert(REM % 16 == 0, "head dims above 64 must be 64*a + 16*b");
   static constexpr int N16 = REM / 16;
   static constexpr int DHP = DH >= 64 ? DH : (DH + 15) / 16 * 16;
@@ -91,10 +98,10 @@
   __host__ __device__ static constexpr int part16_off(int p) { return N64 * P64 + p * P16; }
 };
 
-template <int DH, int ROWS = 128>
+template <int DH, int ROWS = 128, bool NARROW = false>
 __device__ __forceinline__ void tma_load_tile(uint8_t* sdst, const CUtensorMap* map128, const CUtensorMap* map32,
                                               uint64_t* bar, int r0, int h, int b) {
-  using T = TileParts<DH, ROWS>;
+  using T = TileParts<DH, ROWS, NARROW>;
 #pragma unroll
   for (int p = 0; p < T::N64; ++p) tma_load_4d(sdst + T::part64_off(p), map128, bar, p * 64, h, r0, b);
 #pragma unroll
@@ -105,13 +112,16 @@
 __device__ __forceinline__ uint64_t desc_k32(uint32_t part_addr) { return gmma_desc(part_addr, 16, 256, 3); }
 __device__ __forceinline__ uint64_t desc_mn128(uint32_t part_addr, int ks) { return gmma_desc(part_addr + ks * 2048, 16384, 1024, 1); }
 __device__ __forceinline__ uint64_t desc_mn32(uint32_t part_addr, int ks) { return gmma_desc(part_addr + ks * 512, 4096, 256, 3); }
+__device__ __forceinline__ uint64_t desc_mn32_wide(uint32_t part_addr, int ks, uint32_t part_bytes) {
+  return gmma_desc(part_addr + ks * 512, part_bytes, 256, 3);
+}
 
 __host__ __device__ constexpr int align1k(int bytes) { return (bytes + 1023) / 1024 * 1024; }
 
-template <int DH, int AROWS, int BN>
+template <int DH, int AROWS, int BN, bool NARROW = false>
 __device__ __forceinline__ void gemm_kk(float* d, uint32_t sA, int arow0, uint32_t sB) {
-  using TA = TileParts<DH, AROWS>;
-  using TB = TileParts<DH, BN>;
+  using TA = TileParts<DH, AROWS, NARROW>;
+  using TB = TileParts<DH, BN, NARROW>;
   int acc = 0;
 #pragma unroll
   for (int p = 0; p < TA::N64; ++p)
@@ -127,15 +137,20 @@
   }
 }
 
-template <int DH>
+template <int DH, bool NARROW = false>
 struct AccW {
-  using T = TileParts<DH, 64>;
+  using T = TileParts<DH, 64, NARROW>;
   static constexpr int W = T::N64 * 64 + T::N16 * 16;
   static constexpr int REGS = W / 2;
 };
-template <int DH, int KR>
+template <int DH, int KR, bool NARROW = false>
 __device__ __forceinline__ void gemm_rmn(float* d, const uint32_t* a, uint32_t sB) {
-  using TB = TileParts<DH, KR>;
+  using TB = TileParts<DH, KR, NARROW>;
+  if constexpr (NARROW) {
+#pragma unroll
+    for (int ks = 0; ks < KR / 16; ++ks) wgmma_rs<TB::N16 * 16>(d, a + 4 * ks, desc_mn32_wide(sB, ks, TB::P16), 1);
+    return;
+  }
 #pragma unroll
   for (int ks = 0; ks < KR / 16; ++ks) {
 #pragma unroll
```

New measurement: 2.589, median of 6. +2.7%, better.
